# niqbal996/triton_client

Measured on AMD Instinct MI355X. Metric: end-to-end FPS (sensor->detection) YOLOv5n-640 + PointPillars at 1/2/4/8 GPU, higher is better.
Workload: dtype fp32

## Files before the change

triton_client_amd/_native.py:

```python
from __future__ import annotations

import ctypes
import os
import threading
from typing import Optional

from . import _build

_LOCK = threading.Lock()
_KERNELS: Optional[ctypes.CDLL] = None
_RUNTIME: Optional[ctypes.CDLL] = None
_HIP: Optional[ctypes.CDLL] = None

P = ctypes.c_void_p
I = ctypes.c_int
L = ctypes.c_long
F = ctypes.c_float

_KERNEL_SIGS = {
    "tca_draw_boxes": [P, L, I, I, I, I, P, I, I, P, P, I, P],
    "tca_draw_annotations": [P, L, I, I, I, I, P, I, I, P, P, P, I, P, I, P],
    "tca_jpeg_idct": [P, P, P, P, L, L, I, P],
    "tca_jpeg_color": [P, P, P, L, L, I, P],
    "tca_jpeg_fdct": [P, P, P, P, L, L, I, P],
    "tca_jpeg_enc_size": [P, P, P, L, I, P, I, I, P],
    "tca_jpeg_enc_scan": [P, P, I, P, I, P, L, P, I, P],
    "tca_jpeg_enc_write": [P, P, P, L, I, P, I, I, P, L, P, I, P],
    "tca_image_to_rgb8": [P, L, I, I, I, I, I, P, L, I, P],
    "tca_image_preprocess": [P, L, I, I, I, I, I, P, I, I, I, I, I, I, I, I, I, I, F, I, F, F, F, F, F, F, P],
    "tca_c3_fused": [P, P, P],
    "tca_yolo_stem_fused": [P, L, I, I, I, I, I, I, I, I, I, I, I, I, F, I, F, F, F, F, F, F, P, P, I, P, P, I, P, I,
                            I, P],
    "tca_yolo_detect_filter": [P, P, P, P, P, P, P, P, P, I, I, I, F, P, P, P, P, P, P, I, P],
    "tca_yolo_decode": [P, P, P, I, I, I, I, I, P, P, P, P, P, P],
    "tca_yolo_decode_filter": [P, P, P, I, I, I, I, I, P, P, P, P, F, I, P, P, P, P, P, P, I, P, P],
    "tca_yolo_filter_decoded": [P, P, I, I, I, I, I, F, I, P, F, F, P, P, P, P, P, I, P],
    "tca_topk_sort": [P, P, I, I, I, P, P, P],
    "tca_nms_mask": [I, P, I, P, P, P, I, I, I, F, I, P, I, P],
    "tca_nms_mask_rot": [P, I, P, P, P, I, I, I, F, I, P, P, P],
    "tca_nms_reduce": [P, P, P, I, I, P, I, P, P, I, I, P, P, P, P, P, P],
    "tca_box_iou": [P, I, P, I, P, P],
    "tca_box3d_iou": [P, P, P, P, P, P, P, P, P, I, L, P, P, P],
    "tca_points_in_boxes": [P, P, P, I, I, I, I, I, I, I, P, P, P, P, I, P, P, P, P, P],
    "tca_points_in_boxes_chunk": [],
    "tca_bev_render": [P, L, P, P, I, I, I, I, I, I, I, F, F, F, F, F, F, I, I, P, P, P, I, P, I, P, L, I, P],
    "tca_track3d": [P, P, I, P, P, P, I, P, I, I, F, P, P],
    "tca_nms_merge": [P, P, P, P, P, P, P, P, I, I, I, F, I, I, P, P, P, P, P, P],
    "tca_pc2_unpack": [P, P, P, I, I, I, P, P, I, F, P, I, P, P, P, P],
    "tca_pc2_blocks_per_frame": [I],
    "tca_vox_blocks_per_frame": [I],
    "tca_voxelize": [P, I, I, P, I, P, P, P, I, I, I, P, P, P, P, P, P, P, P, P, P, I, I, P, I, P],
    "tca_pillar_vfe_slots": [P, I, I, P, P, P, P, I, I, I, P, P, P, P, I, I, P, P, I, P],
    "tca_pillar_vfe_set_variant": [I],
    "tca_conv_s2sp": [P, I, I, I, I, I, I, P, P, I, P, I, I, I, P, I, P],
    "tca_pillar_vfe_voxels": [P, P, P, P, I, I, I, P, P, P, P, I, I, P, P, I, P],
    "tca_pillar_canvas_clear": [P, P, I, I, I, I, I, P, I, P],
    "tca_pillar_vfe_slots_occ": [P, I, I, P, P, P, P, I, I, I, P, P, P, P, I, I, P, P, I, P, P],
    "tca_pillar_vfe_voxels_occ": [P, P, P, P, I, I, I, P, P, P, P, I, I, P, P, I, P, P],
    "tca_pillar_canvas_clear_occ": [P, P, I, I, I, I, I, P, I, P, P],
    "tca_pillar_occ_clear": [P, P, I, I, I, I, P, P],
    "tca_conv_nhwc": [P, I, I, I, I, I, I, P, P, I, I, I, I, I, I, P, I, I, I, I, I, P, I, I, I, I, P],
    "tca_conv_nhwc_x3": [P, I, I, I, I, I, I, P, P, I, I, I, I, I, I, P, I, I, I, I, I, P, I, I, I, I, P],
    "tca_conv_nhwc_x3p": [P, I, I, I, I, I, I, P, P, I, I, I, I, I, I, P, I, I, I, I, I, P, I, I, I, I, I, P],
    "tca_conv_wino": [P, I, I, I, I, I, I, I, P, P, I, P, I, I, I, I, P, I, P, I, P],
    "tca_conv_hx3p": [P, I, I, I, I, I, I, P, P, I, P, I, I, I, P, I, I, I, P],
    "tca_conv_hx3p_uni": [P, I, I, I, I, I, I, P, P, I, P, I, I, I, P, I, P, I, P],
    "tca_bev_uniform_depth": [P, I, I, I, I, P, P],
    "tca_conv_hx3s2p": [P, I, I, I, I, I, I, P, P, I, P, I, I, I, P, I, I, P, P, I, P, I, P],
    "tca_copy_segments": [I, P, P, P, P],
    "tca_voxel_check": [P, P, P, I, I, I, I, I, I, P, P],
    "tca_sweep_step": [P, I, P, I, I, I, P, P, P, P, P, P, P, ctypes.c_double, P, P, P],
    "tca_planar_affine": [P, I, I, I, P, I, I, F, F, F, F, F, F, P],
    "tca_conv_nhwc_x3p_occ": [P, I, I, I, I, I, I, P, P, I, I, I, I, I, I, P, I, I, I, I, I, P, I, I, I, I, I, P, P],
    "tca_zero_i32": [P, I, P],
    "tca_anchor_decode_filter": [P, P, P, I, I, I, I, I, I, I, I, I, I, I, P, F, F, F, F, F, F, F, P, P, P, P, P, I, P],
    "tca_anchor_decode_filter_keyed": [P, P, P, I, I, I, I, I, I, I, I, I, I, I, P, F, F, F, F, F, F, P, P, P, P, P, P, I,
                                       P],
    "tca_anchor_topk_threshold": [P, I, I, I, I, I, I, I, I, I, P, P, P],
    "tca_pfn2_slots": [P, I, I, P, P, P, P, I, I, I, P, P, P, P, P, P, I, I, P, P, I, P],
    "tca_pfn2_voxels": [P, I, P, P, P, I, I, I, P, P, P, P, P, P, I, I, P, P, I, P],
    "tca_centerhead_decode": [P, I, I, I, I, I, I, P, P, I, F, P, P, I, P, P, P, P, P, P, I, P],
    "tca_maxpool2d_nhwc": [P, I, I, I, I, I, I, I, I, I, P, I, I, I, I, I, P],
    "tca_retina_decode": [P, P, I, I, I, I, I, I, I, I, I, P, F, F, F, F, I, I, P, P, P, P, P, I, I, P],
    "tca_fcos_decode": [P, P, P, I, I, I, I, I, I, I, I, I, F, F, F, I, I, P, P, P, P, P, I, I, P],
    "tca_segment_merge": [P, P, P, P, I, I, P, P, I, I, I, P, P, P, P, P, I, P],
    "tca_group_norm_nhwc": [P, I, I, I, I, I, I, F, P, P, I, P, P, I, I, P],
    "tca_group_norm_nhwc_dt": [P, I, I, I, I, I, I, F, P, P, I, P, P, I, I, I, P],
    "tca_yolov4_decode": [P, P, P, I, I, I, P, P, P, F, F, I, I, P, P, P, P, P, P, P, I, P],
    "tca_sppf_pool3": [P, I, I, I, I, I, I, I, P, I, I, I, I, I, P],
    "tca_maxpool_nhwc": [P, I, I, I, I, I, I, I, P, I, I, I, P],
    "tca_upsample2x_nhwc": [P, I, I, I, I, I, I, P, I, I, I, P],
    "tca_vox_slots_csr": [P, I, P, I, P, P, I, I, P, P, P, P, P, P, P, P, I, P],
    "tca_bev_neck_head": [I, P, P, P, P, P, P, P, P, P, I, P, I, I, I, I, I, P],
    "tca_bev_neck_head_x3": [I, P, P, P, P, P, P, P, P, P, I, P, I, I, I, I, I, P],
    "tca_bev_neck_head_x3p": [I, P, P, P, P, P, P, P, P, P, I, P, I, I, I, I, I, P],
    "tca_bev_neck_head_x3v": [I, P, P, P, P, P, P, P, P, P, I, P, I, I, I, I, I, I, I, P],
    "tca_sp_offsets": [P, I, P, P, P],
    "tca_sp_vfe_slots": [P, I, I, P, P, I, P, P, I, I, P, P, P, P, P, P],
    "tca_sp_vfe_voxels": [P, I, I, I, P, P, P, P, P, P, P, P],
    "tca_sp_claim": [P, P, I, P, P, P, P, P, I, P],
    "tca_sp_rulebook": [P, P, I, P, P, P, P, P, P],
    "tca_sp_grid_reset": [P, P, I, P, P, P],
    "tca_sp_bev_clear": [P, P, I, I, P, I, I, I, P],
    "tca_sp_gemm": [P, I, P, I, P, P, P, I, I, P, I, P, P, P, I, I, I, I, P],
    "tca_sp_vfe_slots_f32": [P, I, I, P, P, I, P, P, I, I, P, P, P, P, P, P],
    "tca_sp_vfe_voxels_f32": [P, I, I, I, P, P, P, P, P, P, P, P],
    "tca_sp_bev_clear_f32": [P, P, I, I, P, I, I, I, P],
    "tca_roi_grid_pool_f32": [P, I, I, I, I, I, I, P, I, P, I, F, F, F, F, I, P, P],
    "tca_sp_gemm_x3": [P, I, P, I, P, P, P, I, I, P, I, P, P, P, I, I, I, I, P],
    "tca_roi_grid_pool": [P, I, I, I, I, I, I, P, I, P, I, F, F, F, F, I, P, P],
    "tca_roi_rescore": [P, P, I, P, P, I, I, F, P, P, P, P, P, P],
}


class NativeError(RuntimeError):
    pass


def _load_hip() -> ctypes.CDLL:
    global _HIP
    if _HIP is None:
        with _LOCK:
            if _HIP is not None:
                return _HIP
            lib = None
            for cand in ("libamdhip64.so", "/opt/rocm/lib/libamdhip64.so"):
                try:
                    lib = ctypes.CDLL(cand)
                    break
                except OSError:
                    continue
            if lib is not None:
                lib.hipGetErrorString.restype = ctypes.c_char_p
                lib.hipGetErrorString.argtypes = [I]
                lib.hipGetLastError.restype = I
                lib.hipGetLastError.argtypes = []
            _HIP = lib
    return _HIP


def _lib_path(name: str) -> str:
    if name == "libtca_kernels.so" and os.environ.get("TCA_KERNELS_LIB"):
        return os.environ["TCA_KERNELS_LIB"]
    return os.path.join(_build.LIBDIR, name)


def kernels(auto_build: bool = True) -> ctypes.CDLL:
    global _KERNELS
    if _KERNELS is not None:
        return _KERNELS
    with _LOCK:
        if _KERNELS is not None:
            return _KERNELS
        path = _lib_path("libtca_kernels.so")
        if not os.path.exists(path) and auto_build:
            _build.build(verbose=False)
        if not os.path.exists(path):
            raise NativeError(f"{path} is missing: run `python -m triton_client_amd._build` (hipcc, gfx950)")
        lib = ctypes.CDLL(path, mode=ctypes.RTLD_GLOBAL)
        for name, args in _KERNEL_SIGS.items():
            fn = getattr(lib, name, None)
            if fn is None:
                if not os.environ.get("TCA_KERNELS_LIB"):
                    raise NativeError(f"{path}: no symbol {name}: rebuild (python -m triton_client_amd._build)")
                continue
            fn.argtypes = args
            fn.restype = I
        _KERNELS = lib
        return lib


def runtime(auto_build: bool = True) -> ctypes.CDLL:
    global _RUNTIME
    if _RUNTIME is not None:
        return _RUNTIME
    with _LOCK:
        if _RUNTIME is not None:
            return _RUNTIME
        path = _lib_path("libtca_runtime.so")
        if not os.path.exists(path) and auto_build:
            _build.build(verbose=False)
        if not os.path.exists(path):
            raise NativeError(f"{path} is missing: run `python -m triton_client_amd._build`")
        lib = ctypes.CDLL(path, mode=ctypes.RTLD_GLOBAL)
        from . import _runtime_sigs
        _runtime_sigs.declare(lib)
        _RUNTIME = lib
        return lib


def check(rc: int, what: str) -> None:
    if rc != 0:
        hip = _load_hip()
        msg = hip.hipGetErrorString(rc).decode() if hip is not None else f"code {rc}"
        raise NativeError(f"{what} failed: {msg} ({rc})")


def call(name: str, *args) -> None:
    fn = getattr(kernels(), name)
    hip = _HIP if _HIP is not None else _load_hip()
    if hip is not None:
        hip.hipGetLastError()
    if args and _KERNEL_SIGS.get(name, [None])[-1] is P and _capturing():
        _check_capture_stream(name, args[-1])
    check(fn(*args), name)


def _capturing() -> bool:
    from .pipelines.graph import capturing_thread
    return capturing_thread()


def _check_capture_stream(name: str, stream) -> None:
    from .pipelines.graph import GraphCaptureError, stream_is_capturing

    h = int(stream or 0)
    if not stream_is_capturing(h):
        raise GraphCaptureError(f"{name}: launched onto stream {hex(h)}, which is not part of the graph being "
                                "captured (its work would not replay)")


def ptr(t) -> int:
    return 0 if t is None else int(t.data_ptr())


def stream_ptr(stream=None) -> int:
    import torch

    s = stream if stream is not None else torch.cuda.current_stream()
    return int(s.cuda_stream)


def available() -> bool:
    try:
        kernels()
        return True
    except Exception:
        return False
```

triton_client_amd/models/fast.py:

```python
from __future__ import annotations

from typing import List, Optional, Sequence, Tuple

import torch
import torch.nn as nn

from .. import _native
from ..ops.conv import NHWC, FusedConv, act_dtype, maxpool_nhwc, sppf_pools, to_pairs, upsample2x_nhwc
from .common import ACT_NONE, ACT_RELU, ACT_SILU, ConvBNAct

STEM_FUSED = True
BEV_UNIFORM = True
WINO_F32_CHAIN = True
DETECT_FUSED = True
C3_FUSED = True
FUSED_C3_WIDTHS = (16, 32, 64)


def bev_out_pair(convs: Sequence[FusedConv], i: int) -> bool:
    if not WINO_F32_CHAIN or i + 1 >= len(convs):
        return True
    return not (convs[i + 1].route(False, False).family == "wino" and convs[i].route(True, False).out_fp32)


def bev_first_conv_gated(cv: FusedConv) -> bool:
    return cv.route(True, True, occ=True).gated


def bev_uniform_eligible(convs: Sequence[FusedConv]) -> bool:
    if not 2 <= len(convs) <= 8:
        return False
    fams = [cv.route(i == 0 or bev_out_pair(convs, i - 1), bev_out_pair(convs, i), occ=i == 0).family
            for i, cv in enumerate(convs)]
    return fams[0] in ("hx3s2", "s2sp") and all(f in ("hx3", "wino") for f in fams[1:])


def _fc(m: ConvBNAct, device, precision: str = "bf16", **kw) -> FusedConv:
    assert m.fused, "call fuse_model() first"
    return FusedConv(m.conv, act=m.act, device=device, precision=precision, **kw)


class _Buffers:
    def __init__(self, device, precision: str = "bf16"):
        self.device = torch.device(device)
        self.precision = precision
        self.dtype = act_dtype(precision) if self.device.type == "cuda" else torch.float32
        self.bufs = []

    def new(self, B, H, W, C, pair: bool = False) -> NHWC:
        t = torch.zeros((B, H, W, C), dtype=self.dtype, device=self.device)
        self.bufs.append(t)
        return NHWC(t, pair=pair)

    def nbytes(self):
        return sum(t.numel() * t.element_size() for t in self.bufs)


def _merged_1x1(a: ConvBNAct, b: ConvBNAct) -> Optional[nn.Conv2d]:
    ca, cb = a.conv, b.conv
    if not (a.fused and b.fused and a.act == b.act and ca.kernel_size == cb.kernel_size == (1, 1)
            and ca.stride == cb.stride == (1, 1) and ca.in_channels == cb.in_channels and ca.groups == cb.groups == 1):
        return None
    m = nn.Conv2d(ca.in_channels, ca.out_channels + cb.out_channels, 1, 1, 0, bias=True)
    with torch.no_grad():
        m.weight.copy_(torch.cat([ca.weight.detach().float(), cb.weight.detach().float()], 0))
        zb = lambda c: c.bias.detach().float() if c.bias is not None else torch.zeros(c.out_channels)
        m.bias.copy_(torch.cat([zb(ca), zb(cb)], 0))
    return m


class _C3Plan:

    def __init__(self, c3, B, H, W, bufs: _Buffers, device):
        pr = bufs.precision
        self.cv1, self.cv2, self.cv3 = _fc(c3.cv1, device, pr), _fc(c3.cv2, device, pr), _fc(c3.cv3, device, pr)
        self.m = [(_fc(b.cv1, device, pr), _fc(b.cv2, device, pr), b.add) for b in c3.m]
        c_ = self.cv1.N
        self.c_ = c_
        mc = _merged_1x1(c3.cv1, c3.cv2) if self.cv1.N == self.cv1.cout_real == self.cv2.N else None
        self.cv12 = FusedConv(mc, act=c3.cv1.act, device=device, precision=pr) if mc is not None else None
        self.cat = bufs.new(B, H, W, 2 * c_)
        self.a = [bufs.new(B, H, W, c_), bufs.new(B, H, W, c_)]
        self.tmp = bufs.new(B, H, W, c_)
        self.out_c = self.cv3.N
        self._fw = None
        convs = [self.cv12, self.cv3] + [c for b1, b2, _ in self.m for c in (b1, b2)] if self.cv12 is not None else []
        if (C3_FUSED and self.cv12 is not None and c_ in FUSED_C3_WIDTHS and torch.device(device).type == "cuda"
                and (len(self.m) == 1 or all(add for _, _, add in self.m)) and (c_ >= 32 or len(self.m) == 1)
                and all(c.precision == "fp32" and not c.transpose and c.act in (0, 1, 2, 3) for c in convs)
                and self.cv12.k == 1 and self.cv12.N == 2 * c_ and self.cv12.cin_p % 32 == 0
                and self.cv3.k == 1 and self.cv3.cin_p == 2 * c_ and self.cv3.N == 2 * c_
                and all(b1.k == 1 and b1.cin_p == c_ and b1.N == c_ and b2.k == 3 and b2.s == 1 and b2.p == 1
                        and b2.cin_p == c_ and b2.N == c_ for b1, b2, _ in self.m)):
            from ..ops.conv import frag_weights
            dev = torch.device(device)
            self._fw = (frag_weights(self.cv12.w_f32_gemm).to(dev), frag_weights(self.cv3.w_f32_gemm).to(dev),
                        [(frag_weights(b1.w_f32_gemm).to(dev), frag_weights(b2.w_f32_gemm).to(dev))
                         for b1, b2, _ in self.m])

    def fused2_ok(self, x: NHWC, out: NHWC) -> bool:
        return (self._fw is not None and C3_FUSED and x.t.is_cuda and not x.pair and not out.pair
                and x.t.dtype == torch.float32 and out.t.dtype == torch.float32 and x.c == self.cv12.cin_p
                and out.c == self.cv3.N and x.off % 4 == 0 and out.off % 4 == 0
                and x.t.shape[-1] % 4 == 0 and out.t.shape[-1] % 4 == 0)

    def _fused2(self, x: NHWC, out: NHWC) -> NHWC:
        import ctypes
        B, H, W, _ = x.shape
        c_, n = self.c_, len(self.m)
        w12, w3, wm = self._fw
        cat_b = (self.cat.t, 2 * c_, c_)

        def launch(mode, i, xin=None, ain=None, bin_=None, y=None, aout=None, bout=None):
            b1, b2, add = self.m[i]
            t = lambda v: v[0] if v is not None else None
            ptrs = [t(xin), t(ain), t(bin_), t(y), t(aout), t(bout), w12, self.cv12.b_gemm, wm[i][0], b1.b_gemm,
                    wm[i][1], b2.b_gemm, w3, self.cv3.b_gemm]
            pa = (ctypes.c_void_p * 14)(*[_native.ptr(p) for p in ptrs])
            ld = lambda v: (v[1], v[2]) if v is not None else (0, 0)
            iv = [mode, c_, self.cv12.cin_p, self.cv3.N, int(bool(add)), B, H, W, *ld(xin), *ld(ain), *ld(bin_),
                  *ld(y), *ld(aout), *ld(bout), self.cv12.act, b1.act, b2.act, self.cv3.act]
            ia = (ctypes.c_int * 24)(*iv)
            _native.call("tca_c3_fused", ctypes.addressof(pa), ctypes.addressof(ia), _native.stream_ptr(None))

        xv, yv = (x.t, x.t.shape[-1], x.off), (out.t, out.t.shape[-1], out.off)
        if n == 1:
            launch(0, 0, xin=xv, y=yv)
            return out
        av = [(t.t, c_, 0) for t in self.a]
        launch(1, 0, xin=xv, aout=av[0], bout=cat_b)
        for i in range(1, n - 1):
            launch(2, i, ain=av[(i - 1) % 2], aout=av[i % 2])
        launch(3, n - 1, ain=av[(n - 2) % 2], bin_=cat_b, y=yv)
        return out

    def __call__(self, x: NHWC, out: NHWC) -> NHWC:
        c_ = self.c_
        if self.fused2_ok(x, out):
            return self._fused2(x, out)
        if self.cv12 is not None:
            self.cv12(x, out=NHWC(self.cat.t, 0, 2 * c_))
            cur = NHWC(self.cat.t, 0, c_)
        else:
            cur = self.cv1(x, out=self.a[0])
        for i, (b1, b2, add) in enumerate(self.m):
            last = i == len(self.m) - 1
            dst = NHWC(self.cat.t, 0, c_) if last else self.a[(i + 1) % 2]
            u = b1(cur, out=self.tmp)
            b2(u, out=dst, res=cur if add else None)
            cur = dst
        if self.cv12 is None:
            self.cv2(x, out=NHWC(self.cat.t, c_, c_))
        return self.cv3(self.cat, out=out)


class FastYOLOv5:
    IN_CHANNELS = 8

    def __init__(self, model, batch: int, img_hw: Tuple[int, int] = (640, 640), device="cuda", s2d: bool = True,
                 precision: str = "bf16"):
        self.device = torch.device(device)
        self.precision = pr = precision
        H, W = img_hw
        self.H, self.W = H, W
        B = batch
        bufs = self.bufs = _Buffers(self.device, precision)
        m = model
        self.s2d = s2d and H % 2 == 0 and W % 2 == 0 and m.b0.conv.kernel_size == (6, 6) \
            and m.b0.conv.stride == (2, 2) and m.b0.conv.padding == (2, 2)
        if self.s2d:
            from ..ops.image import s2d_stem_weight

            assert m.b0.fused, "call fuse_model() first"
            c0 = m.b0.conv
            stem = nn.Conv2d(16, c0.out_channels, 3, 1, 1, bias=True)
            with torch.no_grad():
                stem.weight.copy_(s2d_stem_weight(c0.weight.detach().float()))
                stem.bias.copy_(c0.bias.detach().float() if c0.bias is not None else torch.zeros(c0.out_channels))
            self.x = bufs.new(B, H // 2, W // 2, 16)
            self.b0 = FusedConv(stem, act=m.b0.act, device=device, precision=pr)
        else:
            self.x = bufs.new(B, H, W, self.IN_CHANNELS)
            self.b0 = _fc(m.b0, device, pr, cin_pad=self.IN_CHANNELS)
        self.b1, self.b3, self.b5, self.b7 = (_fc(getattr(m, n), device, pr) for n in ("b1", "b3", "b5", "b7"))
        h2, w2 = H // 2, W // 2
        s4, s8, s16, s32 = (H // 4, W // 4), (H // 8, W // 8), (H // 16, W // 16), (H // 32, W // 32)
        self.t0 = bufs.new(B, h2, w2, self.b0.N)
        self.t1 = bufs.new(B, *s4, self.b1.N)
        self.c3_2 = _C3Plan(m.b2, B, *s4, bufs, device)
        self.t2 = bufs.new(B, *s4, self.c3_2.out_c)
        self.t3 = bufs.new(B, *s8, self.b3.N)
        self.c3_4 = _C3Plan(m.b4, B, *s8, bufs, device)
        c_p3 = self.c3_4.out_c
        self.h14 = _fc(m.h14, device, pr)
        self.cat17 = bufs.new(B, *s8, self.h14.N + c_p3)
        self.p3 = NHWC(self.cat17.t, self.h14.N, c_p3)
        self.t5 = bufs.new(B, *s16, self.b5.N)
        self.c3_6 = _C3Plan(m.b6, B, *s16, bufs, device)
        c_p4 = self.c3_6.out_c
        self.h10 = _fc(m.h10, device, pr)
        self.cat13 = bufs.new(B, *s16, self.h10.N + c_p4)
        self.p4 = NHWC(self.cat13.t, self.h10.N, c_p4)
        self.t7 = bufs.new(B, *s32, self.b7.N)
        self.c3_8 = _C3Plan(m.b8, B, *s32, bufs, device)
        self.t8 = bufs.new(B, *s32, self.c3_8.out_c)
        self.sp1, self.sp2 = _fc(m.b9.cv1, device, pr), _fc(m.b9.cv2, device, pr)
        cs = self.sp1.N
        self.spcat = bufs.new(B, *s32, 4 * cs)
        self.t9 = bufs.new(B, *s32, self.sp2.N)
        self.k = m.b9.k
        self.h18, self.h21 = _fc(m.h18, device, pr), _fc(m.h21, device, pr)
        self.cat23 = bufs.new(B, *s32, self.h21.N + self.h10.N)
        self.h10_out = NHWC(self.cat23.t, self.h21.N, self.h10.N)
        self.c3_13 = _C3Plan(m.h13, B, *s16, bufs, device)
        self.t13 = bufs.new(B, *s16, self.c3_13.out_c)
        self.cat20 = bufs.new(B, *s16, self.h18.N + self.h14.N)
        self.h14_out = NHWC(self.cat20.t, self.h18.N, self.h14.N)
        self.c3_17 = _C3Plan(m.h17, B, *s8, bufs, device)
        self.o3 = bufs.new(B, *s8, self.c3_17.out_c)
        self.c3_20 = _C3Plan(m.h20, B, *s16, bufs, device)
        self.o4 = bufs.new(B, *s16, self.c3_20.out_c)
        self.c3_23 = _C3Plan(m.h23, B, *s32, bufs, device)
        self.o5 = bufs.new(B, *s32, self.c3_23.out_c)
        self.det = [FusedConv(c, act=ACT_NONE, device=device, precision=pr) for c in m.detect]
        self.dout = [bufs.new(B, *s, d.N) for s, d in zip((s8, s16, s32), self.det)]
        self.no_real = m.detect[0].out_channels

    def stem_fused_ok(self) -> bool:
        b0, b1 = self.b0, self.b1
        return (STEM_FUSED and self.s2d and self.precision == "fp32" and b0.N == 16 and b0.cin_p == 16
                and b0.Kp == 160 and b0.k == 3 and b0.s == 1 and b1.cin_p == 16 and b1.N == 32 and b1.Kp == 160
                and b1.k == 3 and b1.s == 2 and b1.p == 1 and not self.t1.pair
                and self.H % 4 == 0 and self.W % 4 == 0 and b0.act in (0, 1, 2, 3) and b1.act in (0, 1, 2, 3))

    def input_view(self) -> torch.Tensor:
        if self.s2d:
            raise RuntimeError("space-to-depth input: use set_input()")
        return self.x.t.permute(0, 3, 1, 2)

    def set_input(self, x: torch.Tensor) -> None:
        if (x.is_cuda and x.dtype == torch.float32 and x.is_contiguous() and self.x.t.is_contiguous()
                and self.x.t.shape[-1] in (8, 16)):
            from ..ops.image import planar_affine

            planar_affine(x, self.x.t)
            return
        if self.s2d:
            from ..ops.image import space_to_depth2

            self.x.t.copy_(space_to_depth2(x.permute(0, 2, 3, 1).to(self.x.t.device)).to(self.x.t.dtype))
        else:
            self.x.t.zero_()
            self.x.t[..., :3].copy_(x.permute(0, 2, 3, 1))

    def detect_fused_ok(self) -> bool:
        return (DETECT_FUSED and self.precision == "fp32" and self.device.type == "cuda"
                and all(d.k == 1 and d.s == 1 and d.p == 0 and not d.transpose and d.act == ACT_NONE
                        and d.cin_p in (64, 128, 256) and d.K == d.Kp and d.N == 256
                        and d.w_gemm.shape == (256, 2 * d.cin_p) and o.c == d.cin_p and not o.pair
                        for d, o in zip(self.det, (self.o3, self.o4, self.o5))))

    def forward(self, from_t1: bool = False, heads: bool = True) -> List[NHWC]:
        if from_t1:
            t = self.t1
        else:
            t = self.b0(self.x, out=self.t0)
            t = self.b1(t, out=self.t1)
        t = self.c3_2(t, out=self.t2)
        t = self.b3(t, out=self.t3)
        p3 = self.c3_4(t, out=self.p3)
        t = self.b5(p3, out=self.t5)
        p4 = self.c3_6(t, out=self.p4)
        t = self.b7(p4, out=self.t7)
        t = self.c3_8(t, out=self.t8)
        cs = self.sp1.N
        y0 = self.sp1(t, out=NHWC(self.spcat.t, 0, cs))
        sppf_pools(y0, self.spcat.t, cs, self.k)
        t9 = self.sp2(self.spcat, out=self.t9)
        h10 = self.h10(t9, out=self.h10_out)
        upsample2x_nhwc(h10, NHWC(self.cat13.t, 0, self.h10.N))
        t13 = self.c3_13(self.cat13, out=self.t13)
        h14 = self.h14(t13, out=self.h14_out)
        upsample2x_nhwc(h14, NHWC(self.cat17.t, 0, self.h14.N))
        o3 = self.c3_17(self.cat17, out=self.o3)
        self.h18(o3, out=NHWC(self.cat20.t, 0, self.h18.N))
        o4 = self.c3_20(self.cat20, out=self.o4)
        self.h21(o4, out=NHWC(self.cat23.t, 0, self.h21.N))
        o5 = self.c3_23(self.cat23, out=self.o5)
        if not heads:
            return [o3, o4, o5]
        outs = []
        for d, o, dst in zip(self.det, (o3, o4, o5), self.dout):
            d(o, out=dst)
            outs.append(NHWC(dst.t, 0, self.no_real))
        return outs


class _BEVBackbonePlan:

    def __init__(self, bb, B: int, ny: int, nx: int, bufs: _Buffers, device, pair: bool = False):
        self.blocks = []
        H, W = ny, nx
        pr = bufs.precision
        convs_all = [[_fc(c, device, pr) for c in blk] for blk in bb.blocks]
        ups_all = [FusedConv(u.conv, act=ACT_RELU, device=device, precision=pr) for u in bb.deblocks]
        self.pair = pair and torch.device(device).type == "cuda" and all(
            c.pair_ok() for c in [cv for blk in convs_all for cv in blk] + ups_all)
        for convs in convs_all:
            s = convs[0].s
            H, W = (H + 2 - 3) // s + 1, (W + 2 - 3) // s + 1
            pp = [bufs.new(B, H, W, convs[0].N, self.pair), bufs.new(B, H, W, convs[0].N, self.pair)]
            self.blocks.append((convs, pp, H, W))
        self.ups = []
        up_c = [u.conv.out_channels for u in bb.deblocks]
        s0 = bb.deblocks[0].s
        if s0 < 1:
            k = int(round(1 / s0))
            H0, W0 = self.blocks[0][2] // k, self.blocks[0][3] // k
        else:
            H0, W0 = self.blocks[0][2] * int(round(s0)), self.blocks[0][3] * int(round(s0))
        self.out_hw = (H0, W0)
        self.cat = bufs.new(B, H0, W0, sum(up_c), self.pair)
        off = 0
        for u, fc, c in zip(bb.deblocks, ups_all, up_c):
            assert u.fused, "call fuse_model() first"
            self.ups.append((fc, off, c))
            off += c
        self.ny, self.nx = ny, nx
        self.uni_vals = self._uniform_values(device) if BEV_UNIFORM else None
        self.depth = None
        if self.uni_vals is not None:
            _, _, H1, W1 = self.blocks[0]
            self.depth = torch.zeros((B, H1, W1), dtype=torch.uint8, device=device)

    def out_pair(self, convs, i: int) -> bool:
        return not self.pair or bev_out_pair(convs, i)

    def _uniform_eligible(self) -> bool:
        return self.pair and bev_uniform_eligible(self.blocks[0][0])

    @torch.no_grad()
    def _uniform_values(self, device) -> Optional[List[torch.Tensor]]:
        if not self._uniform_eligible() or torch.cuda.is_current_stream_capturing():
            return None
        convs = self.blocks[0][0]
        x = NHWC(torch.zeros((1, self.ny, self.nx, convs[0].cin_p), dtype=torch.float32, device=device), pair=True,
                 occ=torch.zeros((1, self.ny, self.nx), dtype=torch.uint8, device=device))
        vals = []
        for i, cv in enumerate(convs):
            Ho, Wo = cv.out_hw(x.t.shape[1], x.t.shape[2])
            x = cv(x, out=NHWC(torch.zeros((1, Ho, Wo, cv.N), dtype=torch.float32, device=device),
                               pair=self.out_pair(convs, i)))
            vals.append(x.t[0, Ho // 2, Wo // 2].clone())
        torch.cuda.synchronize(device)
        return vals

    def forward_blocks(self, canvas: NHWC, stop: Optional[int] = None, outs: Optional[List[NHWC]] = None,
                       mark: Optional[tuple] = None) -> List[NHWC]:
        outs = list(outs or [])
        x = outs[-1] if outs else canvas
        first = len(outs)
        stop = len(self.blocks) if stop is None else stop
        uni = (first == 0 and self.uni_vals is not None and canvas is not None and canvas.occ is not None
               and BEV_UNIFORM)
        if uni:
            B, ny, nx = canvas.occ.shape
            assert (ny, nx) == (self.ny, self.nx) and B == self.depth.shape[0], (canvas.occ.shape, self.depth.shape)
            _native.call("tca_bev_uniform_depth", _native.ptr(canvas.occ), B, ny, nx, len(self.blocks[0][0]),
                         _native.ptr(self.depth), _native.stream_ptr(None))
        issued = sum(len(c) for c, _, _, _ in self.blocks[:first])
        for bi, (convs, pp, H, W) in enumerate(self.blocks):
            if bi < first or bi >= stop:
                continue
            for i, cv in enumerate(convs):
                u = (self.depth, i + 1, self.uni_vals[i]) if uni and bi == 0 else None
                o = pp[i % 2] if self.out_pair(convs, i) else NHWC(pp[i % 2].t, pair=False)
                x = cv(x, out=o, uni=u)
                issued += 1
                if mark is not None and issued == mark[0]:
                    mark[1].record()
            outs.append(x)
        return outs

    def convs_before(self, n_blocks: int) -> int:
        return sum(len(c) for c, _, _, _ in self.blocks[:n_blocks])

    def up_strides(self, bb) -> List[float]:
        return [float(u.s) for u in bb.deblocks]

    def forward(self, canvas: NHWC) -> NHWC:
        for x, (up, off, c) in zip(self.forward_blocks(canvas), self.ups):
            up(x, out=self.cat.slice(off, c))
        return self.cat


class FastBEV:

    def __init__(self, model, batch: int, device="cuda", fused_neck: bool = True,
                 bev_hw: Optional[Tuple[int, int]] = None, precision: str = "bf16", pair: bool = True):
        self.device = torch.device(device)
        self.precision = precision
        cfg = model.cfg
        if bev_hw is not None:
            ny, nx = bev_hw
        else:
            nx, ny, _ = cfg.voxel.grid_size
        B = batch
        bufs = self.bufs = _Buffers(self.device, precision)
        self.bb = _BEVBackbonePlan(model.backbone, B, ny, nx, bufs, device, pair=pair and precision == "fp32")
        self.pair = self.bb.pair
        self.canvas_pairs = None
        self.blocks, self.ups, self.cat, self.out_hw = self.bb.blocks, self.bb.ups, self.bb.cat, self.bb.out_hw
        H0, W0 = self.out_hw
        hd = model.head
        merged = nn.Conv2d(hd.conv_cls.in_channels,
                           hd.conv_cls.out_channels + hd.conv_box.out_channels + hd.conv_dir.out_channels, 1)
        with torch.no_grad():
            merged.weight.copy_(torch.cat([hd.conv_cls.weight, hd.conv_box.weight, hd.conv_dir.weight]).float())
            merged.bias.copy_(torch.cat([hd.conv_cls.bias, hd.conv_box.bias, hd.conv_dir.bias]).float())
        self.head = FusedConv(merged, act=ACT_NONE, device=device, precision=precision)
        self.n_cls, self.n_box, self.n_dir = (hd.conv_cls.out_channels, hd.conv_box.out_channels,
                                              hd.conv_dir.out_channels)
        self.hout = bufs.new(B, H0, W0, self.head.N)
        if self.pair and not self.head.pair_ok():
            raise ValueError("pair storage: the head conv must take the global_load_lds kernels")
        self.neck = None
        strides = self.bb.up_strides(model.backbone)
        if self.device.type == "cuda" and fused_neck and all(s >= 1 and float(s).is_integer() for s in strides):
            from ..ops.neck import FusedNeckHead, neck_head_supported

            ups = [u for u, _, _ in self.ups]
            si = [int(s) for s in strides]
            cins = [blk[0][-1].N for blk in self.blocks]
            if neck_head_supported(ups, si, cins, self.head, H0, W0):
                self.neck = FusedNeckHead(ups, si, self.head, self.device)

    def first_conv_gated(self) -> bool:
        return self.pair and bev_first_conv_gated(self.blocks[0][0][0])

    def forward(self, canvas: NHWC):
        if self.pair and not canvas.pair:
            if self.canvas_pairs is None or self.canvas_pairs.t.shape != canvas.tensor().shape:
                self.canvas_pairs = NHWC(torch.empty_like(canvas.tensor(), dtype=torch.float32), pair=True)
            self.canvas_pairs.t.copy_(to_pairs(canvas.tensor()))
            canvas = self.canvas_pairs
        elif canvas.pair and not self.pair:
            raise TypeError("pair canvas handed to a plan built without pair storage")
        if self.neck is not None:
            self.neck(self.bb.forward_blocks(canvas), self.hout)
        else:
            self.head(self.bb.forward(canvas), out=self.hout)
        return self.head_maps()

    def forward_blocks(self, canvas: NHWC, stop: Optional[int] = None, mark: Optional[tuple] = None) -> List[NHWC]:
        assert self.neck is not None and canvas.pair == self.pair
        return self.bb.forward_blocks(canvas, stop, mark=mark)

    def forward_neck(self, blocks: List[NHWC]):
        if len(blocks) < len(self.bb.blocks):
            blocks = self.bb.forward_blocks(None, outs=blocks)
        self.neck(blocks, self.hout)
        return self.head_maps()

    def head_maps(self):
        t = self.hout.t
        return (NHWC(t, 0, self.n_cls), NHWC(t, self.n_cls, self.n_box),
                NHWC(t, self.n_cls + self.n_box, self.n_dir))


class FastCenterPoint:

    TASK_STRIDE = 16

    def __init__(self, model, batch: int, device="cuda", precision: str = "bf16"):
        from .centerpoint import HEAD_ORDER

        self.device = torch.device(device)
        self.precision = precision
        cfg = self.cfg = model.cfg
        nx, ny, _ = cfg.voxel.grid_size
        B = batch
        bufs = self.bufs = _Buffers(self.device, precision)
        self.bb = _BEVBackbonePlan(model.backbone, B, ny, nx, bufs, device)
        H0, W0 = self.bb.out_hw
        hd = model.head
        self.shared = _fc(hd.shared, device, precision)
        self.sh = bufs.new(B, H0, W0, self.shared.N)
        names = list(HEAD_ORDER) + ["hm"]
        pre = [t.pre[n] for t in hd.tasks for n in names]
        c_mid = pre[0].conv.out_channels
        big = nn.Conv2d(pre[0].conv.in_channels, c_mid * len(pre), 3, 1, 1)
        with torch.no_grad():
            big.weight.copy_(torch.cat([m.conv.weight for m in pre]).float())
            big.bias.copy_(torch.cat([m.conv.bias for m in pre]).float())
        self.pre = FusedConv(big, act=ACT_RELU, device=device, precision=precision)
        self.mid = bufs.new(B, H0, W0, self.pre.N)
        self.c_task_in = c_mid * len(names)
        self.finals = []
        for t, task in enumerate(hd.tasks):
            outs = [task.out[n] for n in names]
            n_out = sum(o.out_channels for o in outs)
            assert n_out <= self.TASK_STRIDE
            conv = nn.Conv2d(self.c_task_in, self.TASK_STRIDE, 3, 1, 1)
            with torch.no_grad():
                conv.weight.zero_()
                conv.bias.zero_()
                o0 = 0
                for h, o in enumerate(outs):
                    conv.weight[o0:o0 + o.out_channels, h * c_mid:(h + 1) * c_mid] = o.weight.float()
                    conv.bias[o0:o0 + o.out_channels] = o.bias.float()
                    o0 += o.out_channels
            self.finals.append(FusedConv(conv, act=ACT_NONE, device=device, precision=precision))
        self.task_offsets = [t * self.TASK_STRIDE for t in range(len(hd.tasks))]
        self.hout = bufs.new(B, H0, W0, self.TASK_STRIDE * len(hd.tasks))

    def forward(self, canvas: NHWC) -> NHWC:
        cat = self.bb.forward(canvas)
        self.shared(cat, out=self.sh)
        self.pre(self.sh, out=self.mid)
        for t, fc in enumerate(self.finals):
            fc(NHWC(self.mid.t, t * self.c_task_in, self.c_task_in),
               out=NHWC(self.hout.t, t * self.TASK_STRIDE, self.TASK_STRIDE))
        return self.hout


def _conv_out(n, k, s, p):
    return (n + 2 * p - k) // s + 1


class FastDetectron:

    IN_CHANNELS = 8

    def __init__(self, model, batch: int, device="cuda", precision: str = "bf16"):
        from ..ops.conv import FusedConv

        self.device = torch.device(device)
        self.precision = precision
        cfg = self.cfg = model.cfg
        B = self.B = batch
        H, W = cfg.input_hw
        bufs = self.bufs = _Buffers(self.device, precision)
        self.x = bufs.new(B, H, W, self.IN_CHANNELS)
        bb = model.backbone
        P = precision
        self.stem = _fc(bb.stem, device, P, cin_pad=self.IN_CHANNELS)
        h, w = _conv_out(H, 7, 2, 3), _conv_out(W, 7, 2, 3)
        self.stem_out = bufs.new(B, h, w, 64)
        h, w = _conv_out(h, 3, 2, 1), _conv_out(w, 3, 2, 1)
        self.pool = bufs.new(B, h, w, 64)
        self.stages = []
        x_c = 64
        for st in bb.stages:
            blocks = []
            for blk in st:
                c1, c2, c3 = _fc(blk.conv1, device, P), _fc(blk.conv2, device, P), blk.conv3
                s = blk.conv1.s if blk.conv1.s > 1 else blk.conv2.s
                ho, wo = _conv_out(h, 1, s, 0), _conv_out(w, 1, s, 0)
                f3 = FusedConv(c3.conv, act=ACT_RELU, device=device, post_res=True, precision=P)
                sc = _fc(blk.shortcut, device, P) if blk.shortcut is not None else None
                t1, t2 = bufs.new(B, ho, wo, c1.N), bufs.new(B, ho, wo, c2.N)
                sbuf = bufs.new(B, ho, wo, sc.N) if sc is not None else None
                out = bufs.new(B, ho, wo, f3.N)
                blocks.append((c1, c2, f3, sc, t1, t2, sbuf, out))
                h, w, x_c = ho, wo, f3.N
            self.stages.append(blocks)
        fpn = model.fpn
        C = cfg.fpn_channels
        self.lv_hw = [blocks[-1][7].shape[1:3] for blocks in self.stages[1:]]
        self.lat = [_fc(m, device, P) for m in fpn.lateral]
        self.outc = [_fc(m, device, P) for m in fpn.output]
        self.lat_buf = [bufs.new(B, hh, ww, C) for hh, ww in self.lv_hw]
        self.up_buf = [bufs.new(B, hh, ww, C) for hh, ww in self.lv_hw[:2]]
        self.p = [bufs.new(B, hh, ww, C) for hh, ww in self.lv_hw]
        self.p6p7_from_c5 = fpn.p6p7_from_c5
        p6 = fpn.p6.conv
        self.p6 = FusedConv(p6, act=ACT_NONE, device=device, precision=P)
        self.p6r = FusedConv(p6, act=ACT_RELU, device=device, precision=P)
        self.p7 = _fc(fpn.p7, device, P)
        h5, w5 = self.lv_hw[2]
        h6, w6 = _conv_out(h5, 3, 2, 1), _conv_out(w5, 3, 2, 1)
        h7, w7 = _conv_out(h6, 3, 2, 1), _conv_out(w6, 3, 2, 1)
# ... 227 lines not shown
```

Baseline: 5007.

## Fuse chained pointwise convolutions into one MFMA kernel for deep YOLO stages

Adds a HIP kernel that runs two back-to-back 1x1 convolutions in one launch. The intermediate activation stays in shared memory as split bf16 hi/lo pairs, and the matrix work uses three-pass MFMA to keep fp32 accuracy. It is wired into three spots: the C3 cv12 to first bottleneck pair, the cv3 to SPPF cv1 pair, and the SPPF cv2 to h10 pair. This removes launches and global round trips of intermediate tensors at the low-resolution stages. If the kernel rejects its arguments, the code falls back to the separate convolutions, at the cost of extra control-flow complexity.

Measured after the change: 5009 (median of 3 runs). About the same (+0.0%).

```diff
diff --git a/csrc/kernels/pw_chain.hip b/csrc/kernels/pw_chain.hip
--- /dev/null
+++ b/csrc/kernels/pw_chain.hip
@@ -0,0 +1,210 @@
+#include "tca_mfma.h"
+
+namespace {
+
+using namespace tca;
+
+constexpr int kBM = 32;
+
+struct PwArgs {
+  const float* x;
+  float* y1;
+  float* y2;
+  const __bf16 *w1, *w2;
+  const float *b1, *b2;
+  long M;
+  int N1, c0, ldx, x_off, ld1, off1, ld2, off2, act1, act2;
+};
+
+__device__ __forceinline__ void split4(const float* v, uint2& h2, uint2& l2) {
+  __bf16 h[4], l[4];
+#pragma unroll
+  for (int r = 0; r < 4; ++r) split_bf16(v[r], h[r], l[r]);
+  h2 = *reinterpret_cast<const uint2*>(h);
+  l2 = *reinterpret_cast<const uint2*>(l);
+}
+
+template <int FN>
+__device__ __forceinline__ void wload(const __bf16* w, int ng, int ks, int g0, int lane, bf16x8 (&h)[FN],
+                                      bf16x8 (&l)[FN]) {
+#pragma unroll
+  for (int j = 0; j < FN; ++j) {
+    const int g = g0 + j < ng ? g0 + j : ng - 1;
+    const __bf16* p = w + ((long)(ks * ng + g) * 2) * 512 + lane * 8;
+    h[j] = *reinterpret_cast<const bf16x8*>(p);
+    l[j] = *reinterpret_cast<const bf16x8*>(p + 512);
+  }
+}
+
+template <int BM, int K1, int K2>
+__global__ void __launch_bounds__(256, 2) pw_chain_kernel(PwArgs a) {
+  constexpr int FM = BM / 16, FN1 = 4, FN2 = 2, NG2 = 8;
+  constexpr int KS1 = K1 / 32, KS2 = K2 / 32;
+  constexpr int P_BYTES = K2 * BM * 2;
+  constexpr int XH = 4 * BM * 8;
+  constexpr int X_BYTES = 2 * XH * 2;
+  __shared__ __attribute__((aligned(16))) unsigned char smem[2 * P_BYTES + 2 * X_BYTES];
+  __bf16* const yh = reinterpret_cast<__bf16*>(smem);
+  __bf16* const yl = reinterpret_cast<__bf16*>(smem + P_BYTES);
+  __bf16* const xs = reinterpret_cast<__bf16*>(smem + 2 * P_BYTES);
+
+  const int tid = threadIdx.x, lane = tid & 63, wid = tid >> 6;
+  const int fr = lane & 15, fq = lane >> 4;
+  const long m0 = (long)blockIdx.x * BM;
+  const int ng1 = a.N1 >> 4;
+
+  constexpr int XPL = BM * 8 / 256;
+  const float* xg[XPL];
+  int xo[XPL];
+#pragma unroll
+  for (int k = 0; k < XPL; ++k) {
+    const int q = tid + k * 256;
+    const int p = (q >> 6) * 8 + ((q >> 1) & 7), f4 = ((q >> 4) & 3) * 2 + (q & 1);
+    xg[k] = m0 + p < a.M ? a.x + (m0 + p) * a.ldx + a.x_off + f4 * 4 : nullptr;
+    xo[k] = ((f4 >> 1) * BM + p) * 8 + (f4 & 1) * 4;
+  }
+  float4 xr[2][XPL];
+  auto xload = [&](int c, float4 (&r)[XPL]) {
+#pragma unroll
+    for (int k = 0; k < XPL; ++k)
+      r[k] = xg[k] ? *reinterpret_cast<const float4*>(xg[k] + c * 32) : make_float4(0.f, 0.f, 0.f, 0.f);
+  };
+  auto xstore = [&](int buf, const float4 (&r)[XPL]) {
+    __bf16* hb = xs + buf * 2 * XH;
+#pragma unroll
+    for (int k = 0; k < XPL; ++k) {
+      const float v[4] = {r[k].x, r[k].y, r[k].z, r[k].w};
+      uint2 h2, l2;
+      split4(v, h2, l2);
+      *reinterpret_cast<uint2*>(hb + xo[k]) = h2;
+      *reinterpret_cast<uint2*>(hb + XH + xo[k]) = l2;
+    }
+  };
+  auto pfrag = [&](const __bf16* ph, const __bf16* pl, int i, int ch, bf16x8& h, bf16x8& l) {
+    const int o = (ch * BM + i * 16 + fr) * 8;
+    h = *reinterpret_cast<const bf16x8*>(ph + o);
+    l = *reinterpret_cast<const bf16x8*>(pl + o);
+  };
+
+  {
+    const int g0 = wid * FN1;
+    f32x4 acc[FM][FN1];
+#pragma unroll
+    for (int i = 0; i < FM; ++i)
+#pragma unroll
+      for (int j = 0; j < FN1; ++j) acc[i][j] = f32x4{0.f, 0.f, 0.f, 0.f};
+    constexpr int RD = 3;
+    bf16x8 wh[RD][FN1], wl[RD][FN1];
+    xload(0, xr[0]);
+    xload(1, xr[1]);
+#pragma unroll
+    for (int c = 0; c < RD - 1; ++c) wload<FN1>(a.w1, ng1, c, g0, lane, wh[c], wl[c]);
+#pragma unroll
+    for (int c = 0; c < KS1; ++c) {
+      xstore(c & 1, xr[c & 1]);
+      if (c + 2 < KS1) xload(c + 2, xr[c & 1]);
+      if (c + RD - 1 < KS1)
+        wload<FN1>(a.w1, ng1, c + RD - 1, g0, lane, wh[(c + RD - 1) % RD], wl[(c + RD - 1) % RD]);
+      __syncthreads();
+      const __bf16* hb = xs + (c & 1) * 2 * XH;
+#pragma unroll
+      for (int i = 0; i < FM; ++i) {
+        bf16x8 xh, xl;
+        pfrag(hb, hb + XH, i, fq, xh, xl);
+#pragma unroll
+        for (int j = 0; j < FN1; ++j) mfma3(acc[i][j], wh[c % RD][j], wl[c % RD][j], xh, xl);
+      }
+    }
+#pragma unroll
+    for (int j = 0; j < FN1; ++j) {
+      if (g0 + j >= ng1) break;
+      const int n = (g0 + j) * 16 + fq * 4;
+      const float4 bv = a.b1 ? *reinterpret_cast<const float4*>(a.b1 + n) : make_float4(0.f, 0.f, 0.f, 0.f);
+      const int k = n - a.c0;
+#pragma unroll
+      for (int i = 0; i < FM; ++i) {
+        const int p = i * 16 + fr;
+        const float v[4] = {act_fn(acc[i][j][0] + bv.x, a.act1), act_fn(acc[i][j][1] + bv.y, a.act1),
+                            act_fn(acc[i][j][2] + bv.z, a.act1), act_fn(acc[i][j][3] + bv.w, a.act1)};
+        if (a.y1 && m0 + p < a.M)
+          *reinterpret_cast<float4*>(a.y1 + (m0 + p) * a.ld1 + a.off1 + n) = make_float4(v[0], v[1], v[2], v[3]);
+        if (k >= 0 && k < K2) {
+          uint2 h2, l2;
+          split4(v, h2, l2);
+          const int o = ((k >> 3) * BM + p) * 8 + (k & 7);
+          *reinterpret_cast<uint2*>(yh + o) = h2;
+          *reinterpret_cast<uint2*>(yl + o) = l2;
+        }
+      }
+    }
+  }
+
+  {
+    const int g0 = wid * FN2;
+    f32x4 acc[FM][FN2];
+#pragma unroll
+    for (int i = 0; i < FM; ++i)
+#pragma unroll
+      for (int j = 0; j < FN2; ++j) acc[i][j] = f32x4{0.f, 0.f, 0.f, 0.f};
+    bf16x8 wh[3][FN2], wl[3][FN2];
+    wload<FN2>(a.w2, NG2, 0, g0, lane, wh[0], wl[0]);
+    wload<FN2>(a.w2, NG2, 1, g0, lane, wh[1], wl[1]);
+    __syncthreads();
+#pragma unroll
+    for (int ks = 0; ks < KS2; ++ks) {
+      if (ks + 2 < KS2) wload<FN2>(a.w2, NG2, ks + 2, g0, lane, wh[(ks + 2) % 3], wl[(ks + 2) % 3]);
+#pragma unroll
+      for (int i = 0; i < FM; ++i) {
+        bf16x8 xh, xl;
+        pfrag(yh, yl, i, ks * 4 + fq, xh, xl);
+#pragma unroll
+        for (int j = 0; j < FN2; ++j) mfma3(acc[i][j], wh[ks % 3][j], wl[ks % 3][j], xh, xl);
+      }
+    }
+#pragma unroll
+    for (int j = 0; j < FN2; ++j) {
+      const int n = (g0 + j) * 16 + fq * 4;
+      const float4 bv = a.b2 ? *reinterpret_cast<const float4*>(a.b2 + n) : make_float4(0.f, 0.f, 0.f, 0.f);
+#pragma unroll
+      for (int i = 0; i < FM; ++i) {
+        const int p = i * 16 + fr;
+        if (m0 + p < a.M)
+          *reinterpret_cast<float4*>(a.y2 + (m0 + p) * a.ld2 + a.off2 + n) =
+              make_float4(act_fn(acc[i][j][0] + bv.x, a.act2), act_fn(acc[i][j][1] + bv.y, a.act2),
+                          act_fn(acc[i][j][2] + bv.z, a.act2), act_fn(acc[i][j][3] + bv.w, a.act2));
+      }
+    }
+  }
+}
+
+template <int K1, int K2>
+int launch_pw(const PwArgs& a, hipStream_t stream) {
+  const long tiles = (a.M + kBM - 1) / kBM;
+  pw_chain_kernel<kBM, K1, K2><<<(unsigned)tiles, 256, 0, stream>>>(a);
+  return (int)hipGetLastError();
+}
+
+}
+
+TCA_API int tca_pw_chain(const void* const* ptrs, const int* v, hipStream_t stream) {
+  PwArgs a;
+  a.x = (const float*)ptrs[0]; a.y1 = (float*)ptrs[1]; a.y2 = (float*)ptrs[2];
+  a.w1 = (const __bf16*)ptrs[3]; a.b1 = (const float*)ptrs[4];
+  a.w2 = (const __bf16*)ptrs[5]; a.b2 = (const float*)ptrs[6];
+  const int B = v[0], H = v[1], W = v[2], K1 = v[3], K2 = v[6], N2 = v[7];
+  a.N1 = v[4]; a.c0 = v[5]; a.ldx = v[8]; a.x_off = v[9]; a.ld1 = v[10]; a.off1 = v[11];
+  a.ld2 = v[12]; a.off2 = v[13]; a.act1 = v[14]; a.act2 = v[15];
+  if (B < 0 || H < 0 || W < 0) return (int)hipErrorInvalidValue;
+  a.M = (long)B * H * W;
+  if (a.M == 0) return 0;
+  auto al = [](const void* p) { return ((uintptr_t)p & 15) == 0; };
+  auto slice = [](int ld, int off, int c) { return ld > 0 && off >= 0 && !(ld & 3) && !(off & 3) && ld >= off + c; };
+  if (a.M >= (1L << 31) - kBM || (K1 != 256 && K1 != 512) || (K2 != 128 && K2 != 256) || N2 != 128 ||
+      a.N1 < 16 || a.N1 > 256 || (a.N1 & 15) || a.c0 < 0 || (a.c0 & 7) || a.c0 + K2 > a.N1 ||
+      !a.x || !a.y2 || !a.w1 || !a.w2 || !al(a.x) || !al(a.y1) || !al(a.y2) || !al(a.w1) || !al(a.w2) ||
+      !al(a.b1) || !al(a.b2) || !slice(a.ldx, a.x_off, K1) || (a.y1 && !slice(a.ld1, a.off1, a.N1)) ||
+      !slice(a.ld2, a.off2, N2) || a.act1 < 0 || a.act1 > 3 || a.act2 < 0 || a.act2 > 3)
+    return (int)hipErrorInvalidValue;
+  if (K1 == 256) return K2 == 128 ? launch_pw<256, 128>(a, stream) : launch_pw<256, 256>(a, stream);
+  return K2 == 128 ? launch_pw<512, 128>(a, stream) : launch_pw<512, 256>(a, stream);
+}
diff --git a/triton_client_amd/_native.py b/triton_client_amd/_native.py
--- a/triton_client_amd/_native.py
+++ b/triton_client_amd/_native.py
@@ -29,6 +29,7 @@
     "tca_image_to_rgb8": [P, L, I, I, I, I, I, P, L, I, P],
     "tca_image_preprocess": [P, L, I, I, I, I, I, P, I, I, I, I, I, I, I, I, I, I, F, I, F, F, F, F, F, F, P],
     "tca_c3_fused": [P, P, P],
+    "tca_pw_chain": [P, P, P],
     "tca_yolo_stem_fused": [P, L, I, I, I, I, I, I, I, I, I, I, I, I, F, I, F, F, F, F, F, F, P, P, I, P, P, I, P, I,
                             I, P],
     "tca_yolo_detect_filter": [P, P, P, P, P, P, P, P, P, I, I, I, F, P, P, P, P, P, P, I, P],
@@ -197,13 +198,17 @@
 
 
 def call(name: str, *args) -> None:
+    check(call_rc(name, *args), name)
+
+
+def call_rc(name: str, *args) -> int:
     fn = getattr(kernels(), name)
     hip = _HIP if _HIP is not None else _load_hip()
     if hip is not None:
         hip.hipGetLastError()
     if args and _KERNEL_SIGS.get(name, [None])[-1] is P and _capturing():
         _check_capture_stream(name, args[-1])
-    check(fn(*args), name)
+    return fn(*args)
 
 
 def _capturing() -> bool:
diff --git a/triton_client_amd/models/fast.py b/triton_client_amd/models/fast.py
--- a/triton_client_amd/models/fast.py
+++ b/triton_client_amd/models/fast.py
@@ -1,5 +1,6 @@
 from __future__ import annotations
 
+import os
 from typing import List, Optional, Sequence, Tuple
 
 import torch
@@ -15,6 +16,8 @@
 DETECT_FUSED = True
 C3_FUSED = True
 FUSED_C3_WIDTHS = (16, 32, 64)
+PW_CHAIN = os.environ.get("TCA_PW_CHAIN", "1") != "0"
+HIP_INVALID_VALUE = 1
 
 
 def bev_out_pair(convs: Sequence[FusedConv], i: int) -> bool:
@@ -67,6 +70,41 @@
         zb = lambda c: c.bias.detach().float() if c.bias is not None else torch.zeros(c.out_channels)
         m.bias.copy_(torch.cat([zb(ca), zb(cb)], 0))
     return m
+
+
+class _PwChain:
+
+    def __init__(self, first: Optional[FusedConv], second: FusedConv, c0: int, device):
+        self.first, self.second, self.c0 = first, second, c0
+        self._fw = None
+        pw = lambda c: (c.precision == "fp32" and not c.transpose and c.k == 1 and c.s == 1 and c.p == 0
+                        and not c.post_res and c.act in (0, 1, 2, 3) and c.K == c.Kp == c.cin_p)
+        if (PW_CHAIN and first is not None and torch.device(device).type == "cuda" and pw(first) and pw(second)
+                and first.cin_p in (256, 512) and first.N % 16 == 0 and first.N <= 256
+                and second.cin_p in (128, 256) and second.N == 128 and c0 % 8 == 0
+                and c0 + second.cin_p <= first.N):
+            from ..ops.conv import frag_weights
+            dev = torch.device(device)
+            self._fw = (frag_weights(first.w_f32_gemm).to(dev), frag_weights(second.w_f32_gemm).to(dev))
+
+    def __call__(self, x: NHWC, y1: Optional[NHWC], y2: NHWC) -> bool:
+        import ctypes
+        ts = [t for t in (x, y1, y2) if t is not None]
+        if not (PW_CHAIN and self._fw is not None and x.c == self.first.cin_p and y2.c == self.second.N
+                and (y1 is None or y1.c == self.first.N) and x.shape[:3] == y2.shape[:3]
+                and all(t.t.is_cuda and t.t.dtype == torch.float32 and not t.pair and t.occ is None and t.t.is_contiguous()
+                        and t.shape[:3] == x.shape[:3] for t in ts)):
+            return False
+        f, s = self.first, self.second
+        B, H, W, _ = x.shape
+        ld = lambda t: (t.t.shape[-1], t.off) if t is not None else (0, 0)
+        pa = (ctypes.c_void_p * 7)(*[_native.ptr(p) for p in (
+            x.t, None if y1 is None else y1.t, y2.t, self._fw[0], f.b_gemm, self._fw[1], s.b_gemm)])
+        ia = (ctypes.c_int * 16)(B, H, W, f.cin_p, f.N, self.c0, s.cin_p, s.N, *ld(x), *ld(y1), *ld(y2), f.act, s.act)
+        rc = _native.call_rc("tca_pw_chain", ctypes.addressof(pa), ctypes.addressof(ia), _native.stream_ptr(None))
+        if rc != HIP_INVALID_VALUE:
+            _native.check(rc, "tca_pw_chain")
+        return rc == 0
 
 
 class _C3Plan:
@@ -97,6 +135,7 @@
             self._fw = (frag_weights(self.cv12.w_f32_gemm).to(dev), frag_weights(self.cv3.w_f32_gemm).to(dev),
                         [(frag_weights(b1.w_f32_gemm).to(dev), frag_weights(b2.w_f32_gemm).to(dev))
                          for b1, b2, _ in self.m])
+        self._pw12 = _PwChain(self.cv12 if self._fw is None else None, self.m[0][0], 0, device)
 
     def fused2_ok(self, x: NHWC, out: NHWC) -> bool:
         return (self._fw is not None and C3_FUSED and x.t.is_cuda and not x.pair and not out.pair
@@ -135,23 +174,31 @@
         return out
 
     def __call__(self, x: NHWC, out: NHWC) -> NHWC:
-        c_ = self.c_
         if self.fused2_ok(x, out):
             return self._fused2(x, out)
+        return self.cv3(self.body(x), out=out)
+
+    def body(self, x: NHWC) -> NHWC:
+        c_ = self.c_
+        u = None
         if self.cv12 is not None:
-            self.cv12(x, out=NHWC(self.cat.t, 0, 2 * c_))
+            if self._pw12(x, NHWC(self.cat.t, 0, 2 * c_), self.tmp):
+                u = self.tmp
+            else:
+                self.cv12(x, out=NHWC(self.cat.t, 0, 2 * c_))
             cur = NHWC(self.cat.t, 0, c_)
         else:
             cur = self.cv1(x, out=self.a[0])
         for i, (b1, b2, add) in enumerate(self.m):
             last = i == len(self.m) - 1
             dst = NHWC(self.cat.t, 0, c_) if last else self.a[(i + 1) % 2]
-            u = b1(cur, out=self.tmp)
+            if i > 0 or u is None:
+                u = b1(cur, out=self.tmp)
             b2(u, out=dst, res=cur if add else None)
             cur = dst
         if self.cv12 is None:
             self.cv2(x, out=NHWC(self.cat.t, c_, c_))
-        return self.cv3(self.cat, out=out)
+        return self.cat
 
 
 class FastYOLOv5:
@@ -209,6 +256,8 @@
         self.spcat = bufs.new(B, *s32, 4 * cs)
         self.t9 = bufs.new(B, *s32, self.sp2.N)
         self.k = m.b9.k
+        self.pw_sp1 = _PwChain(self.c3_8.cv3, self.sp1, 0, device)
+        self.pw_h10 = _PwChain(self.sp2, self.h10, 0, device)
         self.h18, self.h21 = _fc(m.h18, device, pr), _fc(m.h21, device, pr)
         self.cat23 = bufs.new(B, *s32, self.h21.N + self.h10.N)
         self.h10_out = NHWC(self.cat23.t, self.h21.N, self.h10.N)
@@ -272,12 +321,18 @@
         t = self.b5(p3, out=self.t5)
         p4 = self.c3_6(t, out=self.p4)
         t = self.b7(p4, out=self.t7)
-        t = self.c3_8(t, out=self.t8)
         cs = self.sp1.N
-        y0 = self.sp1(t, out=NHWC(self.spcat.t, 0, cs))
+        y0 = NHWC(self.spcat.t, 0, cs)
+        if self.c3_8.fused2_ok(t, self.t8):
+            self.sp1(self.c3_8(t, out=self.t8), out=y0)
+        else:
+            cat8 = self.c3_8.body(t)
+            if not self.pw_sp1(cat8, None, y0):
+                self.sp1(self.c3_8.cv3(cat8, out=self.t8), out=y0)
         sppf_pools(y0, self.spcat.t, cs, self.k)
-        t9 = self.sp2(self.spcat, out=self.t9)
-        h10 = self.h10(t9, out=self.h10_out)
+        h10 = self.h10_out
+        if not self.pw_h10(self.spcat, None, h10):
+            self.h10(self.sp2(self.spcat, out=self.t9), out=h10)
         upsample2x_nhwc(h10, NHWC(self.cat13.t, 0, self.h10.N))
         t13 = self.c3_13(self.cat13, out=self.t13)
         h14 = self.h14(t13, out=self.h14_out)
```
